# lhoangan/arap_flow

Measured on AMD Instinct MI355X. Metric: ARAP solve+warp frames/sec at 854x480 mesh, higher is better.
Workload: dtype f32; 1 GPU; configs[1]: single 854x480 DAVIS-shaped frame, single-segment mask, fd=1; schedule 19/8/400; segments_per_frame=1, fd=1, parallelism=frames sharded, no collective, grid_vertices_per_frame=409920

## Files before the change

arap_flow_amd/csrc/arap_resident.h:

```cpp
#pragma once
#include <type_traits>
#include "arap_device.h"

namespace arap {

constexpr int RES_WGS = 512;
constexpr int RES_MAX_GROUPS = RES_WGS;
constexpr int RES_THREADS = 256;
constexpr int RES_SLOTS = 9;
constexpr int RES_TILES_PER_WG = RES_SLOTS;
constexpr int RT_X = 32, RT_Y = 8;
constexpr int RES_ZX = 2 * RT_X + 2 * RT_Y;
constexpr int RES_ZG = 2 * RES_ZX;
constexpr int RES_MAX_L = 32000;
static_assert(RT_X * RT_Y == RES_THREADS && RT_Y == 2 * (RES_THREADS / 64), "one vertex per lane, two rows per wavefront");
constexpr int RES_MAX_HALO = RES_TILES_PER_WG * (2 * RT_X + 2 * RT_Y);
constexpr int RES_HALO_PER_THREAD = (RES_MAX_HALO + RES_THREADS - 1) / RES_THREADS;
constexpr int RES_MAX_TILES = RES_WGS * RES_TILES_PER_WG;
constexpr int LROW = RT_X + 2;
constexpr int LROWS = RT_Y + 2;
constexpr int LPLANE = LROW * LROWS;
constexpr int LTILE = 5 * LPLANE;
constexpr int RES_LDS_BYTES = RES_TILES_PER_WG * LTILE * 4
                              + ((RES_MAX_HALO * 8 + 15) / 16) * 16
                              + RES_TILES_PER_WG * 8 + 8 + 384
                              + RES_TILES_PER_WG * RES_ZX * 16;
static_assert(2 * ((RES_LDS_BYTES + 1279) / 1280 * 1280) <= 160 * 1024, "two workgroups per CU");
#ifndef RES_HALO_REG_SLOTS
#define RES_HALO_REG_SLOTS 8
#endif
#ifndef RES_WREG_SLOTS
#define RES_WREG_SLOTS 7
#endif
#ifndef RES_WREG_8
#define RES_WREG_8 4
#endif
#ifndef RES_WREG_9
#define RES_WREG_9 4
#endif
#ifndef RES_WREG_FIT
#define RES_WREG_FIT 9
#endif
#ifndef RES_WREG_FIT_FLAT
#define RES_WREG_FIT_FLAT 9
#endif
#ifndef RES_WPIN
#define RES_WPIN 1
#endif
#ifndef RES_PREG_SLOTS
#define RES_PREG_SLOTS 7
#endif
#ifndef RES_PREG_SLOTS_FLAT
#define RES_PREG_SLOTS_FLAT 7
#endif
#ifndef RES_SWEEP1
#define RES_SWEEP1 1
#endif
#ifndef RES_WREG_8_FLAT
#define RES_WREG_8_FLAT 4
#endif
#ifndef RES_WREG_9_FLAT
#define RES_WREG_9_FLAT RES_WREG_9
#endif
#ifndef RES_FIRST_LOOK
#define RES_FIRST_LOOK 5
#endif
#ifndef RES_FIRST_LOOK_2
#define RES_FIRST_LOOK_2 14
#endif
#ifndef RES_FIRST_LOOK_X
#define RES_FIRST_LOOK_X 20
#endif
#ifndef RES_OWN_LOCAL
#define RES_OWN_LOCAL 1
#endif
#ifndef RES_POLL_SLEEP
#define RES_POLL_SLEEP 1
#endif
constexpr unsigned RES_SPIN_LIMIT = 1u << 18;
#ifndef RES_GRAN_STRIDE
#define RES_GRAN_STRIDE 2
#endif
constexpr int RES_GS = RES_GRAN_STRIDE;
constexpr int RES_GRAN_UNITS = 2 * RES_WGS;
constexpr int RES_GRAN_L1 = 2 * RES_GRAN_UNITS * RES_GS;
constexpr int RES_GRAN2_STRIDE = 16;
constexpr int RES_GRAN2_GROUP = 2 * 8 * RES_GRAN2_STRIDE;
constexpr int RES_GRAN_X = RES_GRAN_L1 + 4 * RES_GRAN2_GROUP;
constexpr int RES_GRAN_PER_LAUNCH = RES_GRAN_X + RES_GRAN_L1;
#ifndef RES_FLAT_MAX_RUNS
#define RES_FLAT_MAX_RUNS 2
#endif

constexpr int RES_SUMS_ANY = 0, RES_SUMS_FLAT = 1, RES_SUMS_COUNT = 2;

struct ResWg {
    int slot;
    int rank;
    int wgs;
    int gran;
};

struct ResDev {
    const int* tilelist;
    const int* ntiles;
    const int* tilepos;
    const int* bandx0;
    unsigned long long* zx;
    int rtX, rtY;
    unsigned long long* gran;
    unsigned* err;
    const ResWg* wgmap;
    int allow_fast;
    int force_fail;
    int flat_runs;
    int nowait;
    int fuse_update;
    unsigned long long* stamps;
};

typedef __attribute__((address_space(1))) unsigned long long gu64;
typedef __attribute__((address_space(1))) unsigned gu32;

__device__ __forceinline__ int border_entry(int x, int y)
{
    return y == 0 ? x : (y == RT_Y - 1 ? RT_X + x : (x == 0 ? 2 * RT_X + y : (x == RT_X - 1 ? 2 * RT_X + RT_Y + y : -1)));
}
__device__ __forceinline__ void st_tagged(unsigned long long* p, unsigned hi , float v, bool fast)
{
    const unsigned long long g = ((unsigned long long)hi << 32) | __float_as_uint(v);
    if (fast) __hip_atomic_store(p, g, __ATOMIC_RELAXED, __HIP_MEMORY_SCOPE_WORKGROUP);
    else __hip_atomic_store(p, g, __ATOMIC_RELAXED, __HIP_MEMORY_SCOPE_AGENT);
}
typedef float v2f_t __attribute__((ext_vector_type(2)));
__device__ __forceinline__ float2 fma2(float2 a, float2 b, float2 c)
{
    const v2f_t r = __builtin_elementwise_fma((v2f_t){a.x, a.y}, (v2f_t){b.x, b.y}, (v2f_t){c.x, c.y});
    return make_float2(r.x, r.y);
}
template <int BITNO>
__device__ __forceinline__ float keep_if(unsigned f, float v)
{
    int m;
    asm("v_bfe_i32 %0, %1, %2, 1" : "=v"(m) : "v"(f), "n"(BITNO));
    return __uint_as_float(__float_as_uint(v) & (unsigned)m);
}

__device__ __forceinline__ double block_sum_uniform(double t)
{
    return __hiloint2double(__builtin_amdgcn_readlane(__double2hiint(t), 3), __builtin_amdgcn_readlane(__double2loint(t), 3));
}

template <bool ONE = false>
__device__ __forceinline__ bool group_sum(double part, unsigned epoch, unsigned long long* gran_group, int rank,
                                          int wgs, float* bcast , unsigned* err, float& out,
                                          bool fast = false, double* out_d = nullptr, bool nowait = false,
                                          unsigned long long* tm = nullptr ,
                                          unsigned long long* tarr = nullptr )
{
    const int wave = threadIdx.x >> 6, lane = threadIdx.x & 63;
    unsigned long long c0 = 0ull, c1;
    if (wave == 0) {
        if (tm) c0 = __builtin_amdgcn_s_memtime();
        if (tarr) *tarr += __builtin_amdgcn_s_memrealtime();
        __builtin_amdgcn_s_setprio(3);
        unsigned long long* buf = gran_group + (size_t)(epoch & 1u) * wgs * RES_GS;
        if ((lane >> 1) == 1) {
            const unsigned long long bits = (unsigned long long)__double_as_longlong(part);
            const unsigned hw = lane == 2 ? (unsigned)bits : (unsigned)(bits >> 32);
            const unsigned long long gv = ((unsigned long long)epoch << 32) | hw;
            if (fast)
                __hip_atomic_store(buf + rank * RES_GS + (lane - 2), gv, __ATOMIC_RELAXED, __HIP_MEMORY_SCOPE_WORKGROUP);
            else
                __hip_atomic_store(buf + rank * RES_GS + (lane - 2), gv, __ATOMIC_RELAXED, __HIP_MEMORY_SCOPE_AGENT);
        }
        part = block_sum_uniform(part);
        double v = 0.0;
        bool ok = false;
        if (tm) { c1 = __builtin_amdgcn_s_memtime(); tm[0] += c1 - c0; c0 = c1; }
        __builtin_amdgcn_s_sleep(RES_FIRST_LOOK);
        const bool own1 = RES_OWN_LOCAL && lane == rank;
        const bool look = ONE && lane < wgs && !own1;
        const double idle = own1 ? part : 0.0;
        const unsigned long long* const q1 = buf + RES_GS * ((ONE && lane < wgs) ? lane : 0);
        for (unsigned spins = 0; spins < RES_SPIN_LIMIT; ++spins) {
            if (tm) tm[3] += 1;
            if (ONE) {
                const unsigned long long lo = __hip_atomic_load(q1, __ATOMIC_RELAXED, __HIP_MEMORY_SCOPE_AGENT);
                const unsigned long long hi = __hip_atomic_load(q1 + 1, __ATOMIC_RELAXED, __HIP_MEMORY_SCOPE_AGENT);
                const bool late = look && ((unsigned)(lo >> 32) != epoch || (unsigned)(hi >> 32) != epoch);
                v = look ? __longlong_as_double((long long)((hi << 32) | (lo & 0xffffffffull))) : idle;
                ok = !__any(late) || nowait;
                if (ok) break;
                if (RES_POLL_SLEEP) __builtin_amdgcn_s_sleep(1);
                continue;
            }
            v = 0.0;
            bool mine_ok = true;
            for (int m = lane; m < wgs; m += 64) {
                const unsigned long long lo = __hip_atomic_load(buf + RES_GS * m, __ATOMIC_RELAXED, __HIP_MEMORY_SCOPE_AGENT);
                const unsigned long long hi =
                    __hip_atomic_load(buf + RES_GS * m + 1, __ATOMIC_RELAXED, __HIP_MEMORY_SCOPE_AGENT);
                const bool own = RES_OWN_LOCAL && m == rank;
                mine_ok = mine_ok && (own || ((unsigned)(lo >> 32) == epoch && (unsigned)(hi >> 32) == epoch));
                v += own ? part : __longlong_as_double((long long)((hi << 32) | (lo & 0xffffffffull)));
            }
            ok = __all(mine_ok) || nowait;
            if (ok) break;
            if (RES_POLL_SLEEP) __builtin_amdgcn_s_sleep(1);
        }
        if (tm) { c1 = __builtin_amdgcn_s_memtime(); tm[1] += c1 - c0; c0 = c1; asm volatile("" : "+v"(v)); }
        v = wave_sum_l63_full(v);
        if (tm) {
            asm volatile("" :: "v"(v));
            c1 = __builtin_amdgcn_s_memtime(); tm[4] += c1 - c0;
        }
        if (lane == 63) {
            *(float2*)(bcast + 2 * (epoch & 1u)) = make_float2((float)v, ok ? 1.0f : 0.0f);
            if (out_d) *out_d = v;
            if (!ok) atomicExch(err, 0xDEAD0000u | (epoch & 0xffffu));
        }
        __builtin_amdgcn_s_setprio(0);
        if (tm) { c1 = __builtin_amdgcn_s_memtime(); tm[2] += c1 - c0; c0 = c1; }
    }
    __syncthreads();
    const float2 bc = *(const float2*)(bcast + 2 * (epoch & 1u));
    out = bc.x;
    if (tm && wave == 0) {
        asm volatile("s_waitcnt lgkmcnt(0)" ::: "memory");
        tm[5] += __builtin_amdgcn_s_memtime() - c0;
    }
    return bc.y != 0.0f;
}

__device__ __forceinline__ bool group_sum_h(double part, unsigned epoch, unsigned long long* gran_group,
                                            unsigned long long* gran2 , int rank, int wgs,
                                            float* bcast, unsigned* err, float& out, bool subfast)
{
    const int wave = threadIdx.x >> 6, lane = threadIdx.x & 63;
    if (wave == 0) {
        __builtin_amdgcn_s_setprio(3);
        const int sub = rank >> 6, srank = rank & 63, nsub = wgs >> 6;
        unsigned long long* buf = gran_group + (size_t)sub * (128 * RES_GS) + (size_t)(epoch & 1u) * (64 * RES_GS);
        part = __hiloint2double(__builtin_amdgcn_readfirstlane(__double2hiint(part)),
                                __builtin_amdgcn_readfirstlane(__double2loint(part)));
        if (lane < 2) {
            const unsigned long long bits = (unsigned long long)__double_as_longlong(part);
            const unsigned hw = lane == 0 ? (unsigned)bits : (unsigned)(bits >> 32);
            const unsigned long long gv = ((unsigned long long)epoch << 32) | hw;
            if (subfast)
                __hip_atomic_store(buf + srank * RES_GS + lane, gv, __ATOMIC_RELAXED, __HIP_MEMORY_SCOPE_WORKGROUP);
            else
                __hip_atomic_store(buf + srank * RES_GS + lane, gv, __ATOMIC_RELAXED, __HIP_MEMORY_SCOPE_AGENT);
        }
        double v = 0.0;
        bool ok = false;
        __builtin_amdgcn_s_sleep(RES_FIRST_LOOK);
        for (unsigned spins = 0; spins < RES_SPIN_LIMIT; ++spins) {
            const unsigned long long lo = __hip_atomic_load(buf + RES_GS * lane, __ATOMIC_RELAXED, __HIP_MEMORY_SCOPE_AGENT);
            const unsigned long long hi = __hip_atomic_load(buf + RES_GS * lane + 1, __ATOMIC_RELAXED, __HIP_MEMORY_SCOPE_AGENT);
            const bool own = RES_OWN_LOCAL && lane == srank;
            v = own ? part : __longlong_as_double((long long)((hi << 32) | (lo & 0xffffffffull)));
            ok = __all(own || ((unsigned)(lo >> 32) == epoch && (unsigned)(hi >> 32) == epoch));
            if (ok) break;
            if (RES_POLL_SLEEP) __builtin_amdgcn_s_sleep(1);
        }
        const double ssub = wave_sum_full(v);
        unsigned long long* buf2 = gran2 + (size_t)(epoch & 1u) * (8 * RES_GRAN2_STRIDE);
        if (ok && srank == 0 && lane < 2) {
            const unsigned long long bits = (unsigned long long)__double_as_longlong(ssub);
            const unsigned hw = lane == 0 ? (unsigned)bits : (unsigned)(bits >> 32);
            __hip_atomic_store(buf2 + sub * RES_GRAN2_STRIDE + lane, ((unsigned long long)epoch << 32) | hw, __ATOMIC_RELAXED,
                               __HIP_MEMORY_SCOPE_AGENT);
        }
        bool ok2 = false;
        v = 0.0;
        if (ok) {
            __builtin_amdgcn_s_sleep(RES_FIRST_LOOK_2);
            for (unsigned spins = 0; spins < RES_SPIN_LIMIT; ++spins) {
                bool mine_ok = true;
                v = 0.0;
                if (lane < nsub) {
                    const unsigned long long lo = __hip_atomic_load(buf2 + RES_GRAN2_STRIDE * lane, __ATOMIC_RELAXED, __HIP_MEMORY_SCOPE_AGENT);
                    const unsigned long long hi = __hip_atomic_load(buf2 + RES_GRAN2_STRIDE * lane + 1, __ATOMIC_RELAXED, __HIP_MEMORY_SCOPE_AGENT);
                    const bool own = RES_OWN_LOCAL && srank == 0 && lane == sub;
                    v = own ? ssub : __longlong_as_double((long long)((hi << 32) | (lo & 0xffffffffull)));
                    mine_ok = own || ((unsigned)(lo >> 32) == epoch && (unsigned)(hi >> 32) == epoch);
                }
                ok2 = __all(mine_ok);
                if (ok2) break;
                if (RES_POLL_SLEEP) __builtin_amdgcn_s_sleep(1);
            }
        }
        v = wave_sum_l63_full(v);
        if (lane == 63) {
            *(float2*)(bcast + 2 * (epoch & 1u)) = make_float2((float)v, ok2 ? 1.0f : 0.0f);
            if (!ok2) atomicExch(err, 0xDEAD8000u | (epoch & 0x7fffu));
        }
        __builtin_amdgcn_s_setprio(0);
    }
    __syncthreads();
    const float2 bc = *(const float2*)(bcast + 2 * (epoch & 1u));
    out = bc.x;
    return bc.y != 0.0f;
}

__device__ __forceinline__ bool group_sum_x(double part, unsigned epoch, unsigned long long* gran_group,
                                            unsigned long long* granx_group, int rank, int wgs, float* bcast, unsigned* err,
                                            float& out, bool subfast)
{
    const int wave = threadIdx.x >> 6, lane = threadIdx.x & 63;
    if (wave == 0) {
        __builtin_amdgcn_s_setprio(3);
        const int sub = rank >> 6, srank = rank & 63, nsub = (wgs + 63) >> 6;
        unsigned long long* bufl = gran_group + (size_t)sub * (128 * RES_GS) + (size_t)(epoch & 1u) * (64 * RES_GS);
        unsigned long long* bufx = granx_group + (size_t)(epoch & 1u) * wgs * RES_GS;
        part = __hiloint2double(__builtin_amdgcn_readfirstlane(__double2hiint(part)),
                                __builtin_amdgcn_readfirstlane(__double2loint(part)));
        if (lane < 4) {
            const unsigned long long bits = (unsigned long long)__double_as_longlong(part);
            const unsigned hw = (lane & 1) == 0 ? (unsigned)bits : (unsigned)(bits >> 32);
            const unsigned long long gv = ((unsigned long long)epoch << 32) | hw;
            if (lane < 2) {
                if (subfast)
                    __hip_atomic_store(bufl + srank * RES_GS + lane, gv, __ATOMIC_RELAXED, __HIP_MEMORY_SCOPE_WORKGROUP);
                else
                    __hip_atomic_store(bufl + srank * RES_GS + lane, gv, __ATOMIC_RELAXED, __HIP_MEMORY_SCOPE_AGENT);
            } else {
                __hip_atomic_store(bufx + rank * RES_GS + (lane & 1), gv, __ATOMIC_RELAXED, __HIP_MEMORY_SCOPE_AGENT);
            }
        }
        double v = 0.0;
        bool ok = false;
        __builtin_amdgcn_s_sleep(RES_FIRST_LOOK_X);
        for (unsigned spins = 0; spins < RES_SPIN_LIMIT; ++spins) {
            v = 0.0;
            bool mine_ok = true;
            for (int r = 0; r < nsub; ++r) {
                if (r * 64 + lane >= wgs) break;
                const unsigned long long* src = r == sub ? bufl + RES_GS * lane : bufx + RES_GS * (r * 64 + lane);
                const unsigned long long lo = __hip_atomic_load(src, __ATOMIC_RELAXED, __HIP_MEMORY_SCOPE_AGENT);
                const unsigned long long hi = __hip_atomic_load(src + 1, __ATOMIC_RELAXED, __HIP_MEMORY_SCOPE_AGENT);
                mine_ok = mine_ok && (unsigned)(lo >> 32) == epoch && (unsigned)(hi >> 32) == epoch;
                v += __longlong_as_double((long long)((hi << 32) | (lo & 0xffffffffull)));
            }
            ok = __all(mine_ok);
            if (ok) break;
            if (RES_POLL_SLEEP) __builtin_amdgcn_s_sleep(1);
        }
        v = wave_sum_l63_full(v);
        if (lane == 63) {
            *(float2*)(bcast + 2 * (epoch & 1u)) = make_float2((float)v, ok ? 1.0f : 0.0f);
            if (!ok) atomicExch(err, 0xDEAD4000u | (epoch & 0x3fffu));
        }
        __builtin_amdgcn_s_setprio(0);
    }
    __syncthreads();
    const float2 bc = *(const float2*)(bcast + 2 * (epoch & 1u));
    out = bc.x;
    return bc.y != 0.0f;
}

__device__ __forceinline__ void halo_append(bool take, unsigned short val, unsigned short* hlist, int* nhalo)
{
    const unsigned long long m = __ballot(take);
    if (m == 0ull) return;
    const int first = __builtin_ctzll(m);
    int base = 0;
    if ((int)(threadIdx.x & 63) == first) base = atomicAdd(nhalo, __popcll(m));
    base = __builtin_amdgcn_readlane(base, first);
    const int before = (int)__builtin_amdgcn_mbcnt_hi((unsigned)(m >> 32), __builtin_amdgcn_mbcnt_lo((unsigned)m, 0u));
    if (take) hlist[base + before] = val;
}

__device__ __forceinline__ double block_sum8(double v, double* wsum ,
                                             unsigned long long* tb = nullptr )
{
    static_assert(RES_THREADS / 64 == 4, "one pair sum and one DPP step add four wavefronts");
    unsigned long long c0 = 0ull, c1;
    if (tb) { c0 = __builtin_amdgcn_s_memtime(); asm volatile("" : "+v"(v)); }
    v = wave_sum_l63_full(v);
    if (tb) { asm volatile("" :: "v"(v)); c1 = __builtin_amdgcn_s_memtime(); tb[0] += c1 - c0; c0 = c1; }
    const int wave = threadIdx.x >> 6, lane = threadIdx.x & 63;
    if (lane == 63) wsum[wave] = v;
    __syncthreads();
    double t = 0.0;
    if (wave == 0) {
        const double a = wsum[lane & 3], b = wsum[(lane & 3) ^ 1];
        if (tb) { asm volatile("s_waitcnt lgkmcnt(0)" ::: "memory"); c1 = __builtin_amdgcn_s_memtime(); tb[1] += c1 - c0; c0 = c1; }
        t = dpp_add_f64_full<0x112, 0xf>(a + b);
        if (tb) { asm volatile("" :: "v"(t)); c1 = __builtin_amdgcn_s_memtime(); tb[2] += c1 - c0; }
    }
    return t;
}

template <bool STAMPS, int NS, int SUMS>
__global__ __launch_bounds__(RES_THREADS, 2) void k_pcg_resident(PlanDev pd, ResDev rd, int L)
{
    static_assert(NS >= 1 && NS <= RES_SLOTS, "slots");
    static_assert(SUMS == RES_SUMS_ANY || SUMS == RES_SUMS_FLAT, "group-sum flavour");
    constexpr bool FLAT = SUMS == RES_SUMS_FLAT;
    constexpr bool SPEND = FLAT && !STAMPS;
    constexpr bool ONE_TRIP = FLAT && RES_SWEEP1 != 0;
    constexpr bool PREG = NS <= (FLAT ? RES_PREG_SLOTS_FLAT : RES_PREG_SLOTS);
    constexpr int WFIT = SPEND ? RES_WREG_FIT_FLAT : RES_WREG_FIT;
    unsigned long long tA = 0, tS1 = 0, tB = 0, tS2 = 0, tU = 0, t0 = 0, t1 = 0;
    unsigned long long tm[6] = {0, 0, 0, 0, 0, 0}, tbs = 0, tzr = 0;
    unsigned long long tbp[3] = {0, 0, 0}, tarr[2] = {0, 0};
#define RES_STAMP(acc) do { if (STAMPS) { t1 = __builtin_amdgcn_s_memrealtime(); acc += t1 - t0; t0 = t1; } } while (0)
    extern __shared__ __attribute__((aligned(16))) float lds[];
    const ResWg me = rd.wgmap[blockIdx.x];
    if (me.slot < 0) return;
    const int rank = me.rank;
    if (rd.force_fail) {
        if (threadIdx.x == 0) atomicExch(rd.err, 0xDEADFFFFu);
        return;
    }
    if (__hip_atomic_load(rd.err, __ATOMIC_RELAXED, __HIP_MEMORY_SCOPE_AGENT) != 0u) return;
    const int b = me.slot;
    const int wgs = me.wgs;
    const int W = pd.W, H = pd.H;
    const size_t gb = (size_t)b * pd.N;
    const int tid = threadIdx.x, lane = tid & 63, wave = tid >> 6;
    const int lx = lane & (RT_X - 1), ly = (wave << 1) | (lane >> 5);
    unsigned short* hlist = (unsigned short*)(lds + RES_TILES_PER_WG * LTILE);
    int2* tbase = (int2*)((char*)hlist + ((RES_MAX_HALO * 8 + 15) / 16) * 16);
    float* moLUT = (float*)(tbase + RES_TILES_PER_WG + 1);
    float* bcast = moLUT + 12;
    int* nhalo = (int*)(bcast + 4);
    double* wsum = (double*)(bcast + 6);
    unsigned* nbits = (unsigned*)(wsum + 10);
    unsigned* nremote = nbits + 16;
    float4* zst = (float4*)((char*)lds + RES_LDS_BYTES - RES_TILES_PER_WG * RES_ZX * 16);
    unsigned long long* gran_group = rd.gran + me.gran;
    unsigned long long* granx_group = FLAT ? nullptr : rd.gran + RES_GRAN_X + me.gran;

    const int nt = rd.ntiles[b];
    const int tbase_n = nt / wgs, textra = nt - tbase_n * wgs;
    const int tp = tbase_n + (rank < textra ? 1 : 0);
    const int tfirst = rank * tbase_n + (rank < textra ? rank : textra);
    const int* tl = rd.tilelist + (size_t)b * RES_MAX_TILES;
    float wr2, wf2;
    {
        const Slot sl = pd.slots[b];
        wr2 = sl.wr * sl.wr;
        wf2 = sl.wf * sl.wf;
        if (tid < 10) {
            const int deg = tid % 5, fit = tid / 5;
            float dO = 0.f;
            for (int k = 0; k < deg; ++k) dO = dO + (sl.wr * sl.wr + sl.wr * sl.wr);
            if (fit) dO = fmaf(sl.wf, sl.wf, dO);
            moLUT[tid] = ginv(dO);
        }
        if (tid == 0) { *nhalo = 0; *nremote = 0u; }
        if (tid < 16) nbits[tid] = 0u;
    }

    float rx[NS], ry[NS], ra[NS];
    float dx_[NS], dy_[NS], da_[NS];
    float apx[NS], apy[NS], apa[NS];
    float ma_[NS], mo_[NS];
    float2 pxy[PREG ? NS : 1];
    float pal[PREG ? NS : 1];
    float zx_[PREG ? NS : 1], zy_[PREG ? NS : 1], za_[PREG ? NS : 1];
    unsigned fl[NS];
    int ibase[NS];
    constexpr int NWR = NS <= RES_WREG_SLOTS ? 4 : (NS == 8 ? (SPEND ? RES_WREG_8_FLAT : RES_WREG_8)
                                                            : (SPEND ? RES_WREG_9_FLAT : RES_WREG_9));
    constexpr bool WREG = NWR > 0;
    constexpr bool WPIN = WREG && RES_WPIN != 0;
    float we[WREG ? NS : 1][5];
    const int loff = lx + W * ly;

    const int cell = (ly + 1) * LROW + (lx + 1);
#define TP2(T) ((float2*)(T))
#define TCS(T) ((float2*)(T) + LPLANE)
#define TPA(T) ((T) + 4 * LPLANE)

    int org_[NS];
#pragma unroll
    for (int j = 0; j < NS; ++j) org_[j] = j < tp ? tl[tfirst + j] : -1;
    unsigned long long* const zx_b = rd.zx + (size_t)b * RES_MAX_TILES * RES_ZG;
    for (int c = tid; c < tp * RES_ZG; c += RES_THREADS)
        __hip_atomic_store(zx_b + (size_t)tfirst * RES_ZG + c, 0ull, __ATOMIC_RELAXED, __HIP_MEMORY_SCOPE_AGENT);
    float2 qC[NS], qR[NS], vR[NS], vC[NS], hR[NS], hC[NS];
    float qRa[NS], qM[NS], vRa[NS], vM[NS], hRa[NS], hM[NS];
    unsigned qF[NS], vF[NS], hF[NS];
    const int vrow = ly == 0 ? 0 : RT_Y + 1, hcol = lx == 0 ? 0 : RT_X + 1;
#pragma unroll
    for (int j = 0; j < NS; ++j) {
        qC[j] = qR[j] = vR[j] = vC[j] = hR[j] = hC[j] = make_float2(0.f, 0.f);
        qRa[j] = qM[j] = vRa[j] = vM[j] = hRa[j] = hM[j] = 0.f;
        qF[j] = vF[j] = hF[j] = 0u;
        const int org = org_[j];
        const int y0 = org / W, x0 = org - y0 * W;
        const int x = x0 + lx, y = y0 + ly;
        if (org >= 0 && x < W && y < H) {
            const size_t i = gb + (size_t)(x + W * y);
            qF[j] = pd.flags[i];
            qC[j] = pd.cs[i];
            qR[j] = pd.rO[i]; qRa[j] = pd.rA[i]; qM[j] = pd.preA[i];
            if ((ly == 0 && y0 > 0) || (ly == RT_Y - 1 && y + 1 < H)) {
                const size_t hi = ly == 0 ? i - W : i + W;
                vF[j] = pd.flags[hi]; vR[j] = pd.rO[hi]; vRa[j] = pd.rA[hi]; vM[j] = pd.preA[hi]; vC[j] = pd.cs[hi];
            }
            if ((lx == 0 && x0 > 0) || (lx == RT_X - 1 && x + 1 < W)) {
                const size_t hi = lx == 0 ? i - 1 : i + 1;
                hF[j] = pd.flags[hi]; hR[j] = pd.rO[hi]; hRa[j] = pd.rA[hi]; hM[j] = pd.preA[hi]; hC[j] = pd.cs[hi];
            }
        }
    }
    for (int c = tid; c < NS * LTILE; c += RES_THREADS) lds[c] = 0.f;
    __syncthreads();
#pragma unroll
    for (int j = 0; j < NS; ++j) {
        dx_[j] = dy_[j] = da_[j] = 0.f;
        apx[j] = apy[j] = apa[j] = 0.f;
        const int org = org_[j];
        int x0 = -1, y0 = -1;
        if (org >= 0) { y0 = org / W; x0 = org - y0 * W; }
        float* T = lds + j * LTILE;
        const bool act = (qF[j] & F_ACT) != 0u;
        rx[j] = act ? qR[j].x : 0.f; ry[j] = act ? qR[j].y : 0.f; ra[j] = act ? qRa[j] : 0.f;
        ma_[j] = act ? qM[j] : 0.f;
        mo_[j] = moLUT[__popc(qF[j] & 15u) + 5 * (int)((qF[j] >> 4) & 1u)];
        const float2 p0 = make_float2(mo_[j] * rx[j], mo_[j] * ry[j]);
        const float pa0 = ma_[j] * ra[j];
        if (act) {
            TP2(T)[cell] = p0;
            TCS(T)[cell] = qC[j];
            TPA(T)[cell] = pa0;
        }
        if (PREG) {
            pxy[j] = act ? p0 : make_float2(0.f, 0.f);
            pal[j] = act ? pa0 : 0.f;
        }
        if (vF[j] & F_ACT) {
            const int hc = vrow * LROW + (lx + 1);
            const float mo = moLUT[__popc(vF[j] & 15u) + 5 * (int)((vF[j] >> 4) & 1u)];
            TP2(T)[hc] = make_float2(mo * vR[j].x, mo * vR[j].y); TCS(T)[hc] = vC[j]; TPA(T)[hc] = vM[j] * vRa[j];
        }
        if (hF[j] & F_ACT) {
            const int hc = (ly + 1) * LROW + hcol;
            const float mo = moLUT[__popc(hF[j] & 15u) + 5 * (int)((hF[j] >> 4) & 1u)];
            TP2(T)[hc] = make_float2(mo * hR[j].x, mo * hR[j].y); TCS(T)[hc] = hC[j]; TPA(T)[hc] = hM[j] * hRa[j];
        }
        fl[j] = qF[j];
        ibase[j] = __builtin_amdgcn_readfirstlane(x0 + W * y0);
        if (tid == 0) tbase[j] = make_int2(x0, y0);
    }
    float rho = read_scalar(pd.red + ((size_t)b * pd.nslots + 0) * NSHARD);
    __syncthreads();
#pragma unroll
    for (int j = 0; j < NS; ++j) {
        const unsigned f = fl[j];
        if (WREG) {
            if (NWR > 0) we[j][0] = keep_if<0>(f, wr2);
            if (NWR > 1) we[j][1] = keep_if<1>(f, wr2);
            if (NWR > 2) we[j][2] = keep_if<2>(f, wr2);
            if (NWR > 3) we[j][3] = keep_if<3>(f, wr2);
            if (NS <= WFIT) we[j][4] = keep_if<4>(f, wf2);
        }
        halo_append(ly == 0 && (f & F_E3), (unsigned short)(j * LPLANE + 0 * LROW + lx + 1), hlist, nhalo);
        halo_append(ly == RT_Y - 1 && (f & F_E2), (unsigned short)(j * LPLANE + (RT_Y + 1) * LROW + lx + 1), hlist, nhalo);
        halo_append(lx == 0 && (f & F_E1), (unsigned short)(j * LPLANE + (ly + 1) * LROW + 0), hlist, nhalo);
        halo_append(lx == RT_X - 1 && (f & F_E0), (unsigned short)(j * LPLANE + (ly + 1) * LROW + RT_X + 1), hlist, nhalo);
    }
    __syncthreads();
    const int nh = *nhalo;
    uint2* htab = (uint2*)hlist;
    constexpr bool HREG = NS <= RES_HALO_REG_SLOTS;
    uint2 hreg[RES_HALO_PER_THREAD];
    {
        uint2 e[RES_HALO_PER_THREAD];
#pragma unroll
        for (int u = 0; u < RES_HALO_PER_THREAD; ++u) {
            const int c = tid + u * RES_THREADS;
            e[u] = make_uint2(0u, 0u);
            if (c < nh) {
                const int id = hlist[c];
                const int k = id / LPLANE, rem = id - k * LPLANE;
                const int row = rem / LROW, col = rem - row * LROW;
                const int2 tb = tbase[k];
                const int gx = tb.x + col - 1, gy = tb.y + row - 1;
                e[u].y = (unsigned)(k * (LTILE / 2) + rem) | ((unsigned)(k * LTILE + 4 * LPLANE + rem) << 16);
                const int band = gy / RT_Y;
                const int kx = (gx - rd.bandx0[(size_t)b * rd.rtY + band]) / RT_X;
                const int pos = rd.tilepos[((size_t)b * rd.rtY + band) * rd.rtX + (kx < 0 ? 0 : (kx < rd.rtX ? kx : rd.rtX - 1))];
                const int nfull = textra * (tbase_n + 1);
                const int owner = pos < nfull ? pos / (tbase_n + 1) : textra + (pos - nfull) / (tbase_n > 0 ? tbase_n : 1);
                if (pos >= 0 && owner != rank) atomicOr(&nbits[(owner >> 5) & 15], 1u << (owner & 31));
                const int kxc = kx < 0 ? 0 : (kx < rd.rtX ? kx : rd.rtX - 1);
                const int lxo = gx - (rd.bandx0[(size_t)b * rd.rtY + band] + kxc * RT_X), lyo = gy - band * RT_Y;
                const int zpos = border_entry(lxo, lyo);
                (void)row; (void)col;
                e[u].x = (unsigned)((pos < 0 ? 0 : pos) * RES_ZG + 2 * zpos);
            }
        }
        __syncthreads();
#pragma unroll
        for (int u = 0; u < RES_HALO_PER_THREAD; ++u) {
            if (tid + u * RES_THREADS < RES_MAX_HALO) htab[tid + u * RES_THREADS] = e[u];
            hreg[u] = e[u];
        }
    }
    static_assert(RES_TILES_PER_WG * LTILE < 65536 && LTILE % 2 == 0, "halo table packs 16-bit cell offsets");

    unsigned offP[5], offA[5];
    {
        const int dn[5] = {0, 1, -1, LROW, -LROW};
#pragma unroll
        for (int n = 0; n < 5; ++n) {
            offP[n] = (unsigned)(cell + dn[n]) * 8u;
            offA[n] = (unsigned)(cell + dn[n]) * 4u;
            asm volatile("" : "+v"(offP[n]));
            asm volatile("" : "+v"(offA[n]));
        }
    }
    const int zent = border_entry(lx, ly);
    bool alive = true;
    float alpha_last = 0.f;
    asm volatile("s_waitcnt vmcnt(0)" ::: "memory");
    __syncthreads();
    bool fast = false, zfast = false;
    bool hier = false, subfast = false;
    bool hierx = false;
    unsigned long long* const gran2 =
        FLAT ? nullptr : rd.gran + RES_GRAN_L1 + ((((int)(blockIdx.x & 7u) - (me.rank >> 6)) >> 1) & 3) * RES_GRAN2_GROUP;
    {
        const unsigned xcc = __builtin_amdgcn_s_getreg((3 << 11) | (0 << 6) | 20) & 15u;
        float dummy;
        const double mine = (double)xcc + 65536.0 * (double)(xcc * xcc);
        alive = group_sum<ONE_TRIP>(mine, 1u, gran_group, rank, wgs, bcast, rd.err, dummy, false, wsum + 8);
        const double tot = wsum[8];
        const double s2 = floor(tot / 65536.0), s1 = tot - 65536.0 * s2;
        fast = rd.allow_fast && ((double)wgs * s2 == s1 * s1);
        __syncthreads();
        hier = !FLAT && !fast && wgs > 64;
        hierx = hier && (((wgs + 63) >> 6) <= 2 || ((wgs + 63) >> 6) <= rd.flat_runs);
        if (!fast && rd.allow_fast && alive) {
            if (wave == 0) {
                const unsigned long long* buf = gran_group + (size_t)1 * wgs * RES_GS;
                bool remote = false, elsewhere = false;
                for (int m = lane; m < wgs; m += 64) {
                    const bool nb = ((nbits[(m >> 5) & 15] >> (m & 31)) & 1u) != 0u;
                    const bool same_run = hier && (m >> 6) == (rank >> 6);
                    if (nb || same_run) {
                        const unsigned long long lo = __hip_atomic_load(buf + RES_GS * m, __ATOMIC_RELAXED, __HIP_MEMORY_SCOPE_AGENT);
                        const unsigned long long hi = __hip_atomic_load(buf + RES_GS * m + 1, __ATOMIC_RELAXED, __HIP_MEMORY_SCOPE_AGENT);
                        const double val = __longlong_as_double((long long)((hi << 32) | (lo & 0xffffffffull)));
                        const double q2 = floor(val / 65536.0);
                        const bool other = (unsigned)(lo >> 32) != 1u || (unsigned)(hi >> 32) != 1u ||
                                           (unsigned)(val - 65536.0 * q2) != xcc;
                        remote = remote || (nb && other);
                        elsewhere = elsewhere || (same_run && other);
                    }
                }
                const unsigned any_remote = __any(remote) ? 1u : 0u, any_elsewhere = __any(elsewhere) ? 2u : 0u;
                if (lane == 0) *nremote = any_remote | any_elsewhere;
            }
            __syncthreads();
            zfast = (*nremote & 1u) == 0u;
            subfast = !FLAT && hier && (*nremote & 2u) == 0u;
        } else {
            zfast = fast;
        }
        __syncthreads();
    }
#ifndef RES_PRIO_HI
#define RES_PRIO_HI 2
#endif
#ifndef RES_PRIO_TAIL
#define RES_PRIO_TAIL 2
#endif
#define RES_PRIO(J) { if ((J) + RES_PRIO_TAIL >= NS) __builtin_amdgcn_s_setprio(0); else __builtin_amdgcn_s_setprio(RES_PRIO_HI); }
#define RES_PRIO_END() __builtin_amdgcn_s_setprio(0);
    if (STAMPS) t0 = __builtin_amdgcn_s_memrealtime();
    for (int l = 0; l < L && alive; ++l) {
        static_assert(F_E0 == 1u && F_E1 == 2u && F_E2 == 4u && F_E3 == 8u && F_FIT == 16u && F_ACT == 32u, "bit numbers below");
        if (WPIN) {
#pragma unroll
            for (int j = 0; j < NS; ++j)
#pragma unroll
                for (int e_ = 0; e_ < 5; ++e_)
                    if (e_ < NWR || (e_ == 4 && NS <= WFIT)) asm volatile("" : "+v"(we[WREG ? j : 0][e_]));
        }
        double acc = 0.0;
        float2 Lpv[2], Lcs[2], LqO[2][4], Lcn[2][4];
        float Lpa[2], LqA[2][4];
#define RES_LOAD_A(J)                                                                                  \
        {                                                                                              \
            const int s_ = (J) & 1;                                                                    \
            const char* T_ = (const char*)lds + (J) * (LTILE * 4);                                     \
            if (!PREG) Lpv[s_] = *(const float2*)(T_ + offP[0]);                                       \
            Lcs[s_] = *(const float2*)(T_ + offP[0] + LPLANE * 8);                                     \
            if (!PREG) Lpa[s_] = *(const float*)(T_ + offA[0] + LPLANE * 16);                          \
            _Pragma("unroll") for (int n_ = 0; n_ < 2; ++n_) {                                         \
                LqO[s_][n_] = *(const float2*)(T_ + offP[n_ + 1]);                                     \
                Lcn[s_][n_] = *(const float2*)(T_ + offP[n_ + 1] + LPLANE * 8);                        \
                LqA[s_][n_] = *(const float*)(T_ + offA[n_ + 1] + LPLANE * 16);                        \
            }                                                                                          \
        }
#define RES_LOAD_B(J)                                                                                  \
        {                                                                                              \
            const int s_ = (J) & 1;                                                                    \
            const char* T_ = (const char*)lds + (J) * (LTILE * 4);                                     \
            _Pragma("unroll") for (int n_ = 2; n_ < 4; ++n_) {                                         \
                LqO[s_][n_] = *(const float2*)(T_ + offP[n_ + 1]);                                     \
                Lcn[s_][n_] = *(const float2*)(T_ + offP[n_ + 1] + LPLANE * 8);                        \
                LqA[s_][n_] = *(const float*)(T_ + offA[n_ + 1] + LPLANE * 16);                        \
            }                                                                                          \
        }
        RES_LOAD_A(0)
        RES_LOAD_B(0)
#pragma unroll
        for (int j = 0; j < NS; ++j) {
            RES_PRIO(j)
            unsigned f = fl[j];
            asm volatile("" : "+v"(f));
            const int sj = j & 1;
            if (j + 1 < NS) RES_LOAD_A(j + 1)
            __builtin_amdgcn_sched_barrier(0);
            {
                const float2 pv = PREG ? pxy[PREG ? j : 0] : Lpv[sj];
                const float2 csv = Lcs[sj];
                const float pa_ = PREG ? pal[PREG ? j : 0] : Lpa[sj];
                const float ci = csv.x, si = csv.y;
                const float2 pa2 = make_float2(pa_, pa_);
                float2 axy = make_float2(0.f, 0.f);
                float aa = 0.f;
#define RES_EDGE(BITNO, E, NQX, NQY, NHX, NHY, QX, QY)                                                 \
                {                                                                                      \
                    const float2 qO = LqO[sj][E], cn2 = Lcn[sj][E];                                    \
                    const float qA = LqA[sj][E];                                                       \
                    const float cn = cn2.x, sn = cn2.y;                                                \
                    const float w = (BITNO < NWR) ? we[WREG ? j : 0][BITNO] : keep_if<BITNO>(f, wr2);  \
                    const float2 e = pv - qO;                                                          \
                    const float2 t = fma2(make_float2(NQX, NQY), pa2, e);                              \
                    const float2 u = fma2(make_float2(NHX, NHY), make_float2(qA, qA), e + t);          \
                    axy = fma2(make_float2(w, w), u, axy);                                             \
                    aa = fmaf(-w, fmaf(QX, t.x, (QY) * t.y), aa);                                      \
                    (void)cn; (void)sn;                                                                \
                }
                RES_EDGE(0, 0,     -si,  ci,   -sn,  cn,    si, -ci)
                RES_EDGE(1, 1,      si, -ci,    sn, -cn,   -si,  ci)
                __builtin_amdgcn_sched_barrier(0);
                if (j + 1 < NS) RES_LOAD_B(j + 1)
                __builtin_amdgcn_sched_barrier(0);
                RES_EDGE(2, 2,     -ci, -si,   -cn, -sn,    ci,  si)
                RES_EDGE(3, 3,      ci,  si,    cn,  sn,   -ci, -si)
#undef RES_EDGE
                {
                    const float wf = (WREG && NS <= WFIT) ? we[WREG ? j : 0][4] : keep_if<4>(f, wf2);
                    axy = fma2(make_float2(wf, wf), pv, axy);
                }
                const float ax = axy.x, ay = axy.y;
                apx[j] = ax; apy[j] = ay; apa[j] = aa;
                acc += (double)dot3(pv.x, pv.y, pa_, ax, ay, aa);
            }
            __builtin_amdgcn_sched_barrier(0);
        }
#undef RES_LOAD_A
#undef RES_LOAD_B
        float sigma;
        RES_PRIO_END()
        RES_STAMP(tA);
        {
            const unsigned long long cb = STAMPS ? __builtin_amdgcn_s_memtime() : 0ull;
            const double bs = block_sum8(acc, wsum, STAMPS ? tbp : nullptr);
            if (STAMPS) tbs += __builtin_amdgcn_s_memtime() - cb;
            alive = (!FLAT && hierx) ? group_sum_x(block_sum_uniform(bs), 2u * l + 2u, gran_group, granx_group, rank, wgs, bcast, rd.err, sigma, subfast)
                  : (!FLAT && hier)  ? group_sum_h(block_sum_uniform(bs), 2u * l + 2u, gran_group, gran2, rank, wgs, bcast, rd.err, sigma, subfast)
                          : group_sum<ONE_TRIP>(bs, 2u * l + 2u, gran_group, rank, wgs, bcast, rd.err, sigma, fast, nullptr, rd.nowait != 0,
                                      STAMPS ? tm : nullptr, STAMPS ? tarr : nullptr);
        }
        asm volatile("" : "+v"(sigma));
        if (!alive) break;
        RES_STAMP(tS1);
        float alpha = 0.f;
        if (sigma > 0.f) alpha = rho / sigma;
        acc = 0.0;
        const unsigned ztag = 2u * l + 3u;
#pragma unroll
        for (int j = 0; j < NS; ++j) {
            RES_PRIO(j)
            unsigned f = fl[j];
            asm volatile("" : "+v"(f));
            const float mo = mo_[j], ma = ma_[j];
            rx[j] = fmaf(-alpha, apx[j], rx[j]);
            ry[j] = fmaf(-alpha, apy[j], ry[j]);
            ra[j] = fmaf(-alpha, apa[j], ra[j]);
            const float zx = mo * rx[j], zy = mo * ry[j], za = ma * ra[j];
            if (PREG) { zx_[j] = zx; zy_[j] = zy; za_[j] = za; }
            if (zent >= 0) {
                zst[j * RES_ZX + zent] = make_float4(zx, zy, za, zy);
            }
            acc += (double)keep_if<5>(f, dot3(zx, zy, za, rx[j], ry[j], ra[j]));
            __builtin_amdgcn_sched_barrier(0);
        }
        float rhoNew;
        RES_PRIO_END()
        RES_STAMP(tB);
        {
            const unsigned long long cb = STAMPS ? __builtin_amdgcn_s_memtime() : 0ull;
            const double bs = block_sum8(acc, wsum, STAMPS ? tbp : nullptr);
            if (STAMPS) tbs += __builtin_amdgcn_s_memtime() - cb;
            if (wave != 0) {
                unsigned long long* const out = zx_b + (size_t)tfirst * RES_ZG;
                const float2* const st2 = (const float2*)zst;
                const unsigned sh = (tid & 1) ? 16u : 0u;
                static_assert(((RES_THREADS - 64) & 1) == 0, "a thread keeps the parity of its granules");
                if (zfast) {
                    for (int g = tid - 64; g < tp * RES_ZG; g += RES_THREADS - 64) {
                        const float2 v = st2[g];
                        st_tagged(out + g, (ztag << 16) | ((__float_as_uint(v.y) >> sh) & 0xffffu), v.x, true);
                    }
                } else {
                    for (int g = tid - 64; g < tp * RES_ZG; g += RES_THREADS - 64) {
                        const float2 v = st2[g];
                        st_tagged(out + g, (ztag << 16) | ((__float_as_uint(v.y) >> sh) & 0xffffu), v.x, false);
                    }
                }
            }
            alive = (!FLAT && hierx) ? group_sum_x(block_sum_uniform(bs), 2u * l + 3u, gran_group, granx_group, rank, wgs, bcast, rd.err, rhoNew, subfast)
                  : (!FLAT && hier)  ? group_sum_h(block_sum_uniform(bs), 2u * l + 3u, gran_group, gran2, rank, wgs, bcast, rd.err, rhoNew, subfast)
                          : group_sum<ONE_TRIP>(bs, 2u * l + 3u, gran_group, rank, wgs, bcast, rd.err, rhoNew, fast, nullptr, rd.nowait != 0,
                                      STAMPS ? tm : nullptr, STAMPS ? tarr + 1 : nullptr);
        }
        unsigned long long hg[RES_HALO_PER_THREAD][2];
        unsigned hpk_[HREG ? 1 : RES_HALO_PER_THREAD];
#define RES_HPK(U) (HREG ? hreg[U].y : hpk_[HREG ? 0 : (U)])
#pragma unroll
        for (int u = 0; u < RES_HALO_PER_THREAD; ++u) {
            hg[u][0] = hg[u][1] = (unsigned long long)ztag << 48;
            if (tid + u * RES_THREADS < nh) {
                const unsigned gi = HREG ? hreg[u].x : htab[tid + u * RES_THREADS].x;
                const unsigned long long* q_ = (const unsigned long long*)((const char*)zx_b + (size_t)(gi * 8u));
#pragma unroll
                for (int c = 0; c < 2; ++c) hg[u][c] = __hip_atomic_load(q_ + c, __ATOMIC_RELAXED, __HIP_MEMORY_SCOPE_AGENT);
            }
        }
        if (!alive) break;
        RES_STAMP(tS2);
        float beta = 0.f;
        if (rho > 0.f) beta = rhoNew / rho;
        rho = rhoNew;
        if (l + 1 == L) { alpha_last = alpha; break; }
        float2 hp2[RES_HALO_PER_THREAD];
        float hpa[RES_HALO_PER_THREAD];
        if (PREG) {
#pragma unroll
            for (int j = 0; j < (PREG ? NS : 0); ++j) {
                RES_PRIO(j)
                char* T_ = (char*)lds + j * (LTILE * 4);
                dx_[j] = fmaf(alpha, pxy[j].x, dx_[j]);
                dy_[j] = fmaf(alpha, pxy[j].y, dy_[j]);
                da_[j] = fmaf(alpha, pal[j], da_[j]);
                pxy[j] = make_float2(fmaf(beta, pxy[j].x, zx_[j]), fmaf(beta, pxy[j].y, zy_[j]));
                pal[j] = fmaf(beta, pal[j], za_[j]);
                *(float2*)(T_ + offP[0]) = pxy[j];
                *(float*)(T_ + offA[0] + LPLANE * 16) = pal[j];
            }
        } else {
            float2 Up[NS];
            float Ua[NS];
#pragma unroll
            for (int j = 0; j < NS; ++j) {
                const char* T_ = (const char*)lds + j * (LTILE * 4);
                Up[j] = *(const float2*)(T_ + offP[0]);
                Ua[j] = *(const float*)(T_ + offA[0] + LPLANE * 16);
            }
            __builtin_amdgcn_sched_barrier(0);
#pragma unroll
            for (int j = 0; j < NS; ++j) {
                RES_PRIO(j)
                char* T_ = (char*)lds + j * (LTILE * 4);
                const float mo = mo_[j], ma = ma_[j];
                const float zx = mo * rx[j], zy = mo * ry[j], za = ma * ra[j];
                dx_[j] = fmaf(alpha, Up[j].x, dx_[j]);
                dy_[j] = fmaf(alpha, Up[j].y, dy_[j]);
                da_[j] = fmaf(alpha, Ua[j], da_[j]);
                *(float2*)(T_ + offP[0]) = make_float2(fmaf(beta, Up[j].x, zx), fmaf(beta, Up[j].y, zy));
                *(float*)(T_ + offA[0] + LPLANE * 16) = fmaf(beta, Ua[j], za);
            }
        }
        __builtin_amdgcn_sched_barrier(0);
        {
#pragma unroll
            for (int u = 0; u < RES_HALO_PER_THREAD; ++u) {
                hp2[u] = make_float2(0.f, 0.f); hpa[u] = 0.f;
                if (!HREG) hpk_[u] = 0u;
                if (tid + u * RES_THREADS < nh) {
                    if (!HREG) hpk_[u] = htab[tid + u * RES_THREADS].y;
                    hp2[u] = *(const float2*)((const char*)lds + (RES_HPK(u) & 0xffffu) * 8u);
                    hpa[u] = *(const float*)((const char*)lds + (RES_HPK(u) >> 16) * 4u);
                }
            }
        }
#pragma unroll
        for (int j = 0; j < NS; ++j)
            if (HREG) asm volatile("" : "+v"(dx_[j]), "+v"(dy_[j]), "+v"(da_[j]));
        __builtin_amdgcn_sched_barrier(0);
        {
            bool fresh = true;
#pragma unroll
            for (int u = 0; u < RES_HALO_PER_THREAD; ++u)
#pragma unroll
                for (int c = 0; c < 2; ++c) fresh = fresh && (unsigned)(hg[u][c] >> 48) == ztag;
            if (!__all(fresh) && !rd.nowait) {
                for (unsigned spins = 0; spins < RES_SPIN_LIMIT; ++spins) {
                    if (STAMPS) tzr += 1;
                    fresh = true;
#pragma unroll
                    for (int u = 0; u < RES_HALO_PER_THREAD; ++u) {
                        if (tid + u * RES_THREADS < nh) {
                            const unsigned gi = HREG ? hreg[u].x : htab[tid + u * RES_THREADS].x;
                            const unsigned long long* q_ = (const unsigned long long*)((const char*)zx_b + (size_t)(gi * 8u));
#pragma unroll
                            for (int c = 0; c < 2; ++c) {
                                hg[u][c] = __hip_atomic_load(q_ + c, __ATOMIC_RELAXED, __HIP_MEMORY_SCOPE_AGENT);
                                fresh = fresh && (unsigned)(hg[u][c] >> 48) == ztag;
                            }
                        }
                    }
                    if (__all(fresh)) break;
                    __builtin_amdgcn_s_sleep(1);
                }
                if (!fresh) atomicExch(rd.err, 0xDEAD0000u | (ztag & 0xffffu));
            }
        }
#pragma unroll
        for (int u = 0; u < RES_HALO_PER_THREAD; ++u) {
            const float2 hz2_ = make_float2(__uint_as_float((unsigned)hg[u][0]),
                                            __uint_as_float(((unsigned)(hg[u][0] >> 32) & 0xffffu) | ((unsigned)(hg[u][1] >> 32) << 16)));
            const float hz1_ = __uint_as_float((unsigned)hg[u][1]);
            if (tid + u * RES_THREADS < nh) {
                float2* P = (float2*)((char*)lds + (RES_HPK(u) & 0xffffu) * 8u);
                float* A = (float*)((char*)lds + (RES_HPK(u) >> 16) * 4u);
                *P = make_float2(fmaf(beta, hp2[u].x, hz2_.x), fmaf(beta, hp2[u].y, hz2_.y));
                *A = fmaf(beta, hpa[u], hz1_);
            }
        }
        RES_PRIO_END()
        __syncthreads();
        RES_STAMP(tU);
    }
    if (STAMPS && tid == 0) {
        unsigned long long* o = rd.stamps + (size_t)blockIdx.x * 16;
        o[8] = tbs; o[9] = tm[0]; o[10] = tm[1]; o[11] = tm[2]; o[12] = tm[3]; o[13] = tzr;
        o[0] = tA; o[1] = tS1; o[2] = tB; o[3] = tS2; o[4] = tU; o[5] = (unsigned long long)tp; { unsigned pc = 0; for (int q = 0; q < 16; ++q) pc += __popc(nbits[q]); o[6] = (unsigned long long)nh | ((unsigned long long)pc << 32) | ((unsigned long long)*nremote << 48); } o[7] = (fast ? 1ull : 0ull) | (zfast ? 2ull : 0ull) | (hier ? 4ull : 0ull) | (subfast ? 8ull : 0ull);
        unsigned long long* q = rd.stamps + (size_t)RES_WGS * 16 + (size_t)blockIdx.x * 16;
        q[0] = tbp[0]; q[1] = tbp[1]; q[2] = tbp[2]; q[3] = tm[4]; q[4] = tm[5]; q[5] = tarr[0]; q[6] = tarr[1];
        q[7] = (unsigned long long)__builtin_amdgcn_s_getreg((31 << 11) | (0 << 6) | 4) |
               ((unsigned long long)(__builtin_amdgcn_s_getreg((3 << 11) | (0 << 6) | 20) & 15u) << 32);
        q[8] = (unsigned long long)tp; q[9] = (unsigned long long)nh; q[10] = (unsigned long long)tp * RES_ZG;
        q[11] = (unsigned long long)rank | ((unsigned long long)wgs << 16) | ((unsigned long long)b << 32); q[12] = (unsigned long long)L;
    }
    if (!alive) return;
    if (L > 0) {
#pragma unroll
        for (int j = 0; j < NS; ++j) {
            const char* T_ = (const char*)lds + j * (LTILE * 4);
            const float2 p2 = PREG ? pxy[PREG ? j : 0] : *(const float2*)(T_ + offP[0]);
            const float pa1 = PREG ? pal[PREG ? j : 0] : *(const float*)(T_ + offA[0] + LPLANE * 16);
            dx_[j] = fmaf(alpha_last, p2.x, dx_[j]);
            dy_[j] = fmaf(alpha_last, p2.y, dy_[j]);
            da_[j] = fmaf(alpha_last, pa1, da_[j]);
        }
    }
    int lo = loff;
    asm volatile("" : "+v"(lo));
    if (rd.fuse_update) {
        const Slot sl = pd.slots[b];
        float2 o_[NS];
        float a_[NS];
#pragma unroll
        for (int j = 0; j < NS; ++j) {
            o_[j] = make_float2(0.f, 0.f); a_[j] = 0.f;
            if (fl[j] & F_ACT) { const int i = ibase[j] + lo; o_[j] = sl.O[i]; a_[j] = sl.A[i]; }
        }
#pragma unroll
        for (int j = 0; j < NS; ++j) {
            if (fl[j] & F_ACT) {
                const int i = ibase[j] + lo;
                float2 o = o_[j];
                o.x = o.x + dx_[j];
                o.y = o.y + dy_[j];
                const float a = a_[j] + da_[j];
                sl.O[i] = o;
                sl.A[i] = a;
                pd.cs[gb + i] = sincos_spec(a);
            }
        }
        return;
    }
#pragma unroll
    for (int j = 0; j < NS; ++j) {
        const unsigned f = fl[j];
        if (f & F_ACT) {
            const int i = ibase[j] + lo;
            pd.deltaO[gb + i] = make_float2(dx_[j], dy_[j]);
            pd.deltaA[gb + i] = da_[j];
        }
    }
}

#undef RES_STAMP
#undef RES_HPK
#undef RES_PRIO
#undef RES_PRIO_END
#undef TP2
#undef TCS
#undef TPA

}
```

Baseline: 32.11 frames/s.

## Keep cos/sin and halo search-direction values in registers across PCG iterations

Keeps the per-slot cos/sin pair in VGPRs instead of reloading it from LDS on every matvec. When slot counts are small enough, it also keeps halo search-direction values in registers across iterations, so the halo update no longer reads them back from LDS. It adds in-place FMA asm helpers and adjusts the asm register-pinning barriers. The trade is higher VGPR pressure, which risks spills or lower occupancy at the larger slot counts the thresholds allow.

```diff
diff --git a/arap_flow_amd/csrc/arap_resident.h b/arap_flow_amd/csrc/arap_resident.h
--- a/arap_flow_amd/csrc/arap_resident.h
+++ b/arap_flow_amd/csrc/arap_resident.h
@@ -53,6 +53,18 @@
 #ifndef RES_PREG_SLOTS_FLAT
 #define RES_PREG_SLOTS_FLAT 7
 #endif
+#ifndef RES_CSREG_SLOTS
+#define RES_CSREG_SLOTS 7
+#endif
+#ifndef RES_CSREG_SLOTS_FLAT
+#define RES_CSREG_SLOTS_FLAT 7
+#endif
+#ifndef RES_HPREG_SLOTS
+#define RES_HPREG_SLOTS 6
+#endif
+#ifndef RES_HPREG_SLOTS_FLAT
+#define RES_HPREG_SLOTS_FLAT 7
+#endif
 #ifndef RES_SWEEP1
 #define RES_SWEEP1 1
 #endif
@@ -144,6 +156,19 @@
     int m;
     asm("v_bfe_i32 %0, %1, %2, 1" : "=v"(m) : "v"(f), "n"(BITNO));
     return __uint_as_float(__float_as_uint(v) & (unsigned)m);
+}
+
+template <int BITNO>
+__device__ __forceinline__ float keep_if_here(unsigned f, float v)
+{
+    int m;
+    asm volatile("v_bfe_i32 %0, %1, %2, 1" : "=v"(m) : "v"(f), "n"(BITNO));
+    return __uint_as_float(__float_as_uint(v) & (unsigned)m);
+}
+
+__device__ __forceinline__ void fma_into(float& p, float b, float z)
+{
+    asm("v_fma_f32 %0, %1, %0, %2" : "+v"(p) : "v"(b), "v"(z));
 }
 
 __device__ __forceinline__ double block_sum_uniform(double t)
@@ -403,6 +428,7 @@
     constexpr bool SPEND = FLAT && !STAMPS;
     constexpr bool ONE_TRIP = FLAT && RES_SWEEP1 != 0;
     constexpr bool PREG = NS <= (FLAT ? RES_PREG_SLOTS_FLAT : RES_PREG_SLOTS);
+    constexpr bool CSREG = NS <= (FLAT ? RES_CSREG_SLOTS_FLAT : RES_CSREG_SLOTS) - (STAMPS ? 1 : 0);
     constexpr int WFIT = SPEND ? RES_WREG_FIT_FLAT : RES_WREG_FIT;
     unsigned long long tA = 0, tS1 = 0, tB = 0, tS2 = 0, tU = 0, t0 = 0, t1 = 0;
     unsigned long long tm[6] = {0, 0, 0, 0, 0, 0}, tbs = 0, tzr = 0;
@@ -462,6 +488,7 @@
     float ma_[NS], mo_[NS];
     float2 pxy[PREG ? NS : 1];
     float pal[PREG ? NS : 1];
+    v2f_t csr[CSREG ? NS : 1];
     float zx_[PREG ? NS : 1], zy_[PREG ? NS : 1], za_[PREG ? NS : 1];
     unsigned fl[NS];
     int ibase[NS];
@@ -535,6 +562,7 @@
             pxy[j] = act ? p0 : make_float2(0.f, 0.f);
             pal[j] = act ? pa0 : 0.f;
         }
+        if (CSREG) csr[j] = act ? (v2f_t){qC[j].x, qC[j].y} : (v2f_t){0.f, 0.f};
         if (vF[j] & F_ACT) {
             const int hc = vrow * LROW + (lx + 1);
             const float mo = moLUT[__popc(vF[j] & 15u) + 5 * (int)((vF[j] >> 4) & 1u)];
@@ -675,6 +703,19 @@
 #endif
 #define RES_PRIO(J) { if ((J) + RES_PRIO_TAIL >= NS) __builtin_amdgcn_s_setprio(0); else __builtin_amdgcn_s_setprio(RES_PRIO_HI); }
 #define RES_PRIO_END() __builtin_amdgcn_s_setprio(0);
+    constexpr bool HPREG = HREG && NS <= (FLAT ? RES_HPREG_SLOTS_FLAT : RES_HPREG_SLOTS) - (STAMPS ? 1 : 0);
+    float2 hp2[RES_HALO_PER_THREAD];
+    float hpa[RES_HALO_PER_THREAD];
+    if (HPREG) {
+#pragma unroll
+        for (int u = 0; u < RES_HALO_PER_THREAD; ++u) {
+            hp2[u] = make_float2(0.f, 0.f); hpa[u] = 0.f;
+            if (tid + u * RES_THREADS < nh) {
+                hp2[u] = *(const float2*)((const char*)lds + (hreg[u].y & 0xffffu) * 8u);
+                hpa[u] = *(const float*)((const char*)lds + (hreg[u].y >> 16) * 4u);
+            }
+        }
+    }
     if (STAMPS) t0 = __builtin_amdgcn_s_memrealtime();
     for (int l = 0; l < L && alive; ++l) {
         static_assert(F_E0 == 1u && F_E1 == 2u && F_E2 == 4u && F_E3 == 8u && F_FIT == 16u && F_ACT == 32u, "bit numbers below");
@@ -684,6 +725,10 @@
 #pragma unroll
                 for (int e_ = 0; e_ < 5; ++e_)
                     if (e_ < NWR || (e_ == 4 && NS <= WFIT)) asm volatile("" : "+v"(we[WREG ? j : 0][e_]));
+        }
+        if (CSREG) {
+#pragma unroll
+            for (int j = 0; j < (CSREG ? NS : 0); ++j) asm volatile("" : "+v"(csr[j]));
         }
         double acc = 0.0;
         float2 Lpv[2], Lcs[2], LqO[2][4], Lcn[2][4];
@@ -693,7 +738,7 @@
             const int s_ = (J) & 1;                                                                    \
             const char* T_ = (const char*)lds + (J) * (LTILE * 4);                                     \
             if (!PREG) Lpv[s_] = *(const float2*)(T_ + offP[0]);                                       \
-            Lcs[s_] = *(const float2*)(T_ + offP[0] + LPLANE * 8);                                     \
+            if (!CSREG) Lcs[s_] = *(const float2*)(T_ + offP[0] + LPLANE * 8);                         \
             if (!PREG) Lpa[s_] = *(const float*)(T_ + offA[0] + LPLANE * 16);                          \
             _Pragma("unroll") for (int n_ = 0; n_ < 2; ++n_) {                                         \
                 LqO[s_][n_] = *(const float2*)(T_ + offP[n_ + 1]);                                     \
@@ -717,13 +762,13 @@
         for (int j = 0; j < NS; ++j) {
             RES_PRIO(j)
             unsigned f = fl[j];
-            asm volatile("" : "+v"(f));
+            if (NWR < 4 || !(WREG && NS <= WFIT)) asm volatile("" : "+v"(f));
             const int sj = j & 1;
             if (j + 1 < NS) RES_LOAD_A(j + 1)
             __builtin_amdgcn_sched_barrier(0);
             {
                 const float2 pv = PREG ? pxy[PREG ? j : 0] : Lpv[sj];
-                const float2 csv = Lcs[sj];
+                const float2 csv = CSREG ? make_float2(csr[CSREG ? j : 0].x, csr[CSREG ? j : 0].y) : Lcs[sj];
                 const float pa_ = PREG ? pal[PREG ? j : 0] : Lpa[sj];
                 const float ci = csv.x, si = csv.y;
                 const float2 pa2 = make_float2(pa_, pa_);
@@ -784,8 +829,6 @@
 #pragma unroll
         for (int j = 0; j < NS; ++j) {
             RES_PRIO(j)
-            unsigned f = fl[j];
-            asm volatile("" : "+v"(f));
             const float mo = mo_[j], ma = ma_[j];
             rx[j] = fmaf(-alpha, apx[j], rx[j]);
             ry[j] = fmaf(-alpha, apy[j], ry[j]);
@@ -795,7 +838,7 @@
             if (zent >= 0) {
                 zst[j * RES_ZX + zent] = make_float4(zx, zy, za, zy);
             }
-            acc += (double)keep_if<5>(f, dot3(zx, zy, za, rx[j], ry[j], ra[j]));
+            acc += (double)keep_if_here<5>(fl[j], dot3(zx, zy, za, rx[j], ry[j], ra[j]));
             __builtin_amdgcn_sched_barrier(0);
         }
         float rhoNew;
@@ -846,8 +889,6 @@
         if (rho > 0.f) beta = rhoNew / rho;
         rho = rhoNew;
         if (l + 1 == L) { alpha_last = alpha; break; }
-        float2 hp2[RES_HALO_PER_THREAD];
-        float hpa[RES_HALO_PER_THREAD];
         if (PREG) {
 #pragma unroll
             for (int j = 0; j < (PREG ? NS : 0); ++j) {
@@ -856,8 +897,10 @@
                 dx_[j] = fmaf(alpha, pxy[j].x, dx_[j]);
                 dy_[j] = fmaf(alpha, pxy[j].y, dy_[j]);
                 da_[j] = fmaf(alpha, pal[j], da_[j]);
-                pxy[j] = make_float2(fmaf(beta, pxy[j].x, zx_[j]), fmaf(beta, pxy[j].y, zy_[j]));
-                pal[j] = fmaf(beta, pal[j], za_[j]);
+                asm volatile("" : "+v"(dx_[j]), "+v"(dy_[j]), "+v"(da_[j]), "+v"(pxy[j].x), "+v"(pxy[j].y), "+v"(pal[j]));
+                fma_into(pxy[j].x, beta, zx_[j]);
+                fma_into(pxy[j].y, beta, zy_[j]);
+                fma_into(pal[j], beta, za_[j]);
                 *(float2*)(T_ + offP[0]) = pxy[j];
                 *(float*)(T_ + offA[0] + LPLANE * 16) = pal[j];
             }
@@ -885,7 +928,7 @@
             }
         }
         __builtin_amdgcn_sched_barrier(0);
-        {
+        if (!HPREG) {
 #pragma unroll
             for (int u = 0; u < RES_HALO_PER_THREAD; ++u) {
                 hp2[u] = make_float2(0.f, 0.f); hpa[u] = 0.f;
@@ -899,7 +942,7 @@
         }
 #pragma unroll
         for (int j = 0; j < NS; ++j)
-            if (HREG) asm volatile("" : "+v"(dx_[j]), "+v"(dy_[j]), "+v"(da_[j]));
+            if (HREG && !PREG) asm volatile("" : "+v"(dx_[j]), "+v"(dy_[j]), "+v"(da_[j]));
         __builtin_amdgcn_sched_barrier(0);
         {
             bool fresh = true;
@@ -937,8 +980,16 @@
             if (tid + u * RES_THREADS < nh) {
                 float2* P = (float2*)((char*)lds + (RES_HPK(u) & 0xffffu) * 8u);
                 float* A = (float*)((char*)lds + (RES_HPK(u) >> 16) * 4u);
-                *P = make_float2(fmaf(beta, hp2[u].x, hz2_.x), fmaf(beta, hp2[u].y, hz2_.y));
-                *A = fmaf(beta, hpa[u], hz1_);
+                if (HPREG) {
+                    fma_into(hp2[u].x, beta, hz2_.x);
+                    fma_into(hp2[u].y, beta, hz2_.y);
+                    fma_into(hpa[u], beta, hz1_);
+                    *P = hp2[u];
+                    *A = hpa[u];
+                } else {
+                    *P = make_float2(fmaf(beta, hp2[u].x, hz2_.x), fmaf(beta, hp2[u].y, hz2_.y));
+                    *A = fmaf(beta, hpa[u], hz1_);
+                }
             }
         }
         RES_PRIO_END()
```

Result: faster. 33.60 frames/s (median of 6 runs) (+4.6%).
